# NVIDIA/RAD-MMM

Measured on AMD Instinct MI355X. Metric: mel-frames/sec training step (fwd+bwd), higher is better.
Workload: dtype f32 (f16 hi.hi product + fp8 e4m3 cross terms, fp32 accumulate); 1 GPU; RADTTS flow decoder (configs/RADTTS_model_config.yaml: 8 flows, WN 1024x4, D=1048) fwd+NLL+bwd; batch_per_gpu=32, n_mel=80, frames=800, global_batch=32, parallelism=dp1, includes_optimizer=False

## Files before the change

include/radmmm_hip.h:

```cpp
#ifndef RADMMM_HIP_H
#define RADMMM_HIP_H

#include <stdint.h>

#ifdef __cplusplus
extern "C" {
#endif

#define RADMMM_ABI_VERSION 4

typedef void* radmmm_stream_t;

const char* radmmm_last_error(void);
int radmmm_abi_version(void);

enum { RADMMM_ACT_NONE = 0, RADMMM_ACT_SOFTPLUS = 1, RADMMM_ACT_RELU = 2, RADMMM_ACT_LEAKY = 3 };
enum { RADMMM_SCALE_TANH = 0, RADMMM_SCALE_EXP = 1, RADMMM_SCALE_SIGMOID = 2, RADMMM_SCALE_TRANSLATE = 3 };

#define RADMMM_SPLIT_F16 0
#define RADMMM_SPLIT_X8A 1
#define RADMMM_SPLIT_X8B 2
typedef struct { int fmt; int x8_exp; int32_t* sat_flag;
                 void* lo16;
} radmmm_split_opts;
// ... 82 lines not shown
                        float* gz, int ldz, int rows, int D, int h, radmmm_stream_t stream);

int radmmm_squeeze_rows(const float* in , float* out, int B, int C, int T, int g, int ld, int col0,
                        radmmm_stream_t stream);
int radmmm_unsqueeze_rows(const float* gout, float* gin , int B, int C, int T, int g, int ld, int col0,
                          radmmm_stream_t stream);

int radmmm_affine_coupling_fwd(const float* O, int ldo, const float* z, int ldz,
                               float* zout, float* log_s, int rows, int h, int scaling,
                               radmmm_stream_t stream);
int radmmm_affine_coupling_bwd(const float* O, int ldo, const float* z, int ldz,
                               const float* gzout, const float* glog_s,
                               float* gO, float* gz, int rows, int h, int scaling,
                               radmmm_stream_t stream);

int radmmm_dact_mul(const float* g, int ldg, const float* saved, int lds, float* y, int ldy,
                    int rows, int cols, int dact, int rowscale, int T, const int32_t* lens,
                    int taps, int dil,
                    void* yh, void* yl, int ldyh, float yscale ,
                    const radmmm_split_opts* so , radmmm_stream_t stream);

int radmmm_colsum(const float* X, int ldx, float* out, float* scratch, int rows, int cols,
                  int row_weight, int T, const int32_t* lens, int taps, int dil, int square,
                  radmmm_stream_t stream);
int64_t radmmm_colsum_scratch_floats(int rows, int cols);

int radmmm_masked_reduce(const float* x, int B, int C, int T, int64_t sb, int64_t sc, int64_t st,
                         const int32_t* lens, int mode, float* out, float* scratch,
                         radmmm_stream_t stream);
int64_t radmmm_masked_reduce_scratch_floats(int B, int C, int T);
int radmmm_masked_reduce_bwd(const float* x, int B, int C, int T, int64_t sb, int64_t sc,
                             int64_t st, const int32_t* lens, int mode, const float* coef,
                             float* gx, radmmm_stream_t stream);

int radmmm_fused_add_tanh_sigmoid_multiply(const float* a, const float* b, int ld, float* y,
                                           int ldy, int rows, int n, radmmm_stream_t stream);

int radmmm_pq_spline_fwd(const float* x, int ldx, const float* q, int ldq, float* y, int ldy,
                         float* logj_sum, int rows, int h, int K, radmmm_stream_t stream);
int radmmm_pq_spline_bins(const float* x, int ldx, const float* q, int ldq, int32_t* bins, float* edge_l, float* edge_r,
                          int rows, int h, int K, radmmm_stream_t stream);
int radmmm_pq_spline_inv(const float* y, int ldy, const float* q, int ldq, float* x, int ldx, int rows, int h, int K,
                         radmmm_stream_t stream);
int radmmm_pq_spline_bwd(const float* x, int ldx, const float* q, int ldq, const float* gy,
                         int ldgy, const float* glogj, float* gx, int ldgx, float* gq, int ldgq,
                         int rows, int h, int K, radmmm_stream_t stream);

int radmmm_film_fwd(const float* h2, int ldh, const float* c1, int ldc, const float* x1r, int ldx,
                    const float* mean, const float* invstd, const float* w, const float* b,
                    float* out, int ldo, int rows, int C, int use_bn, radmmm_stream_t stream);
int radmmm_film_bwd(const float* h2, int ldh, const float* c1, int ldc, const float* gout, int ldg,
                    const float* mean, const float* invstd, const float* w, const float* b,
                    float n_valid, int T, const int32_t* lens, float* gh2, int ldgh, float* gc1,
                    int ldgc, float* gx1r, int ldgx, float* gw, float* gb, float* scratch, int rows,
                    int C, int use_bn, radmmm_stream_t stream);
int64_t radmmm_film_bwd_scratch_floats(int rows, int C);
int radmmm_film_bwd_sums(const float* h2, int ldh, const float* c1, int ldc, const float* gout, int ldg,
                         const float* mean, const float* invstd, const float* w, const float* b, float* gw, float* gb,
                         float* scratch, int rows, int C, radmmm_stream_t stream);
int radmmm_film_bwd_apply(const float* h2, int ldh, const float* c1, int ldc, const float* gout, int ldg,
                          const float* mean, const float* invstd, const float* w, const float* b, float n_valid, int T,
                          const int32_t* lens, float* gh2, int ldgh, float* gc1, int ldgc, float* gx1r, int ldgx,
                          const float* scratch, int rows, int C, radmmm_stream_t stream);

int radmmm_attn_fwd(const float* Q, const float* Kx, const float* prior, const int32_t* in_lens,
                    float* attn, float* logprob, int B, int T1, int T2, int Ca, float temp,
// ... 223 lines not shown
```

rad_mmm_amd/_lib.py:

```python
from __future__ import annotations

import ctypes as C
import os
from typing import Optional

import torch

_HERE = os.path.dirname(os.path.abspath(__file__))
LIB_PATH = os.environ.get("RADMMM_LIB_PATH") or os.path.join(_HERE, "libradmmm_hip.so")



def debug_env(name: str, default: Optional[str] = None) -> Optional[str]:
    if os.environ.get("RADMMM_DEBUG", "0") in ("", "0"):
        return default
    return os.environ.get(name, default)


ACT_NONE, ACT_SOFTPLUS, ACT_RELU, ACT_LEAKY = 0, 1, 2, 3
SCALE = {"tanh": 0, "exp": 1, "sigmoid": 2, "translate": 3}
ACT = {"none": 0, "softplus": 1, "relu": 2, "leaky_relu": 3}


class RadmmmError(RuntimeError):
# ... 6 lines not shown
        ("a_item_stride", C.c_int64),
        ("B", C.c_void_p), ("ldb", C.c_int), ("b_tap_stride", C.c_int64), ("b_layout", C.c_int),
        ("C", C.c_void_p), ("ldc", C.c_int),
        ("M", C.c_int), ("N", C.c_int), ("K", C.c_int),
        ("taps", C.c_int), ("dil", C.c_int), ("sign", C.c_int),
        ("T", C.c_int),
        ("lens", C.c_void_p),
        ("a_mask_mode", C.c_int),
        ("bias", C.c_void_p),
        ("pconv", C.c_int), ("premask", C.c_int), ("postmask", C.c_int),
        ("ratio_taps", C.c_int), ("ratio_dil", C.c_int),
        ("add", C.c_void_p), ("ldadd", C.c_int),
        ("dact_src", C.c_void_p), ("lddact", C.c_int), ("dact", C.c_int),
        ("rowscale", C.c_int),
        ("act", C.c_int),
        ("C2", C.c_void_p), ("ldc2", C.c_int), ("c2_accum", C.c_int),
        ("Ch", C.c_void_p), ("Cl", C.c_void_p), ("ldch", C.c_int), ("ch_scale", C.c_float),
        ("C2h", C.c_void_p), ("C2l", C.c_void_p), ("ldc2h", C.c_int), ("c2h_scale", C.c_float),
        ("split_fmt", C.c_int), ("ch_x8_exp", C.c_int), ("c2h_x8_exp", C.c_int),
        ("sat_flag", C.c_void_p),
        ("Clo", C.c_void_p),
        ("colsum_out", C.c_void_p), ("colsum_scratch", C.c_void_p),
        ("dact_h", C.c_void_p), ("dact_x", C.c_void_p), ("lddact_h", C.c_int), ("dact_x8_exp", C.c_int),
        ("c2_src", C.c_void_p * 3), ("n_c2_src", C.c_int),
    ]


class CsItem(C.Structure):
    _fields_ = [("part", C.c_void_p), ("out", C.c_void_p), ("nparts", C.c_int), ("cols", C.c_int)]


class DactItem(C.Structure):
    _fields_ = [("saved", C.c_void_p), ("yh", C.c_void_p), ("yl", C.c_void_p), ("ylo16", C.c_void_p), ("part", C.c_void_p)]


class SplitOpts(C.Structure):
    _fields_ = [("fmt", C.c_int), ("x8_exp", C.c_int), ("sat_flag", C.c_void_p), ("lo16", C.c_void_p)]


SPLIT_F16, SPLIT_X8A, SPLIT_X8B = 0, 1, 2


def split_opts(fmt: int = 0, x8_exp: int = 0, sat_flag: Optional[torch.Tensor] = None, lo16: Optional[torch.Tensor] = None):
    return C.byref(SplitOpts(fmt, x8_exp, sat_flag.data_ptr() if sat_flag is not None else None,
                             lo16.data_ptr() if lo16 is not None else None))


class RowGemmH3Desc(C.Structure):
    _fields_ = [
        ("base", RowGemmDesc),
        ("Ah", C.c_void_p), ("Al", C.c_void_p), ("lda_h", C.c_int),
        ("Bh", C.c_void_p), ("Bl", C.c_void_p), ("ldb_h", C.c_int), ("b_tap_stride_h", C.c_int64),
        ("acc_scale", C.c_float),
        ("nprod", C.c_int),
        ("a8_exp", C.c_int), ("b8_exp", C.c_int),
        ("extra_tap", C.c_int), ("extra_a_rows", C.c_int),
    ]


class WnItem(C.Structure):
    _fields_ = [("v", C.c_void_p), ("g", C.c_void_p), ("Wh", C.c_void_p), ("Wl", C.c_void_p), ("inv_norm", C.c_void_p),
                ("Cout", C.c_int), ("Cin", C.c_int), ("taps", C.c_int), ("ldk", C.c_int), ("perm_split", C.c_int),
                ("off_lo", C.c_int), ("off_hi", C.c_int)]


class TpItem(C.Structure):
# ... 16 lines not shown


def _load() -> C.CDLL:
    if not os.path.exists(LIB_PATH):
        raise ImportError(
            f"{LIB_PATH} not found: build it with `python -c 'import __graft_entry__ as g; g.build()'` "
            "or rad_mmm_amd/csrc/build.sh (hipcc --offload-arch=gfx950). rad_mmm_amd has no fallback path.")
    lib = C.CDLL(LIB_PATH)
    lib.radmmm_last_error.restype = C.c_char_p
    lib.radmmm_abi_version.restype = C.c_int
    lib.radmmm_gemm_cu_slots.restype = C.c_int
    lib.radmmm_gemm_cu_slots.argtypes = []
    if lib.radmmm_abi_version() != 4:
        raise ImportError("libradmmm_hip.so ABI version mismatch")
    i, i64, p = C.c_int, C.c_int64, C.c_void_p
    f = C.c_float
    so = C.POINTER(SplitOpts)
    sig = {
        "radmmm_rowgemm_f32": [C.POINTER(RowGemmDesc), p],
        "radmmm_wgrad_f32": [C.POINTER(WgradDesc), p],
        "radmmm_rowgemm_h3": [C.POINTER(RowGemmH3Desc), p],
        "radmmm_weightnorm_fwd": [p, p, p, p, i, i, i, i, i, i, i, p],
        "radmmm_weightnorm_bwd": [p, p, p, p, i, i64, p, p, i, i, i, i, i, i, i, p, p],
        "radmmm_wn_input_fwd": [p, i, p, i, p, i, i, i, i, p, p, so, p],
        "radmmm_wn_input_bwd": [p, i, p, i, i, p, i, i, i, i, p],
        "radmmm_squeeze_rows": [p, p, i, i, i, i, i, i, p],
        "radmmm_unsqueeze_rows": [p, p, i, i, i, i, i, i, p],
        "radmmm_affine_coupling_fwd": [p, i, p, i, p, p, i, i, i, p],
        "radmmm_affine_coupling_bwd": [p, i, p, i, p, p, p, p, i, i, i, p],
        "radmmm_dact_mul": [p, i, p, i, p, i, i, i, i, i, i, p, i, i, p, p, i, f, so, p],
        "radmmm_colsum": [p, i, p, p, i, i, i, i, p, i, i, i, p],
        "radmmm_masked_reduce": [p, i, i, i, i64, i64, i64, p, i, p, p, p],
        "radmmm_masked_reduce_bwd": [p, i, i, i, i64, i64, i64, p, i, p, p, p],
        "radmmm_fused_add_tanh_sigmoid_multiply": [p, p, i, p, i, i, i, p],
        "radmmm_film_fwd": [p, i, p, i, p, i, p, p, p, p, p, i, i, i, i, p],
        "radmmm_film_bwd": [p, i, p, i, p, i, p, p, p, p, f, i, p, p, i, p, i, p, i, p, p, p, i, i, i, p],
        "radmmm_film_bwd_sums": [p, i, p, i, p, i, p, p, p, p, p, p, p, i, i, p],
        "radmmm_film_bwd_apply": [p, i, p, i, p, i, p, p, p, p, f, i, p, p, i, p, i, p, i, p, i, i, p],
        "radmmm_split_f16": [p, i, p, p, i, i, i, f, so, p],
        "radmmm_transpose_split_act": [p, i, i, i, i, i, i, p, i, f, p, p, p, p, i, p],
        "radmmm_wgrad_h3_tiles": [i, i, i],
        "radmmm_wgrad_rm_tiles": [i, i, i],
        "radmmm_wgrad_rm": [p, p, i, p, p, i, i, i, p, i, p, i, i64, i, i, i, i, i, f, p],
        "radmmm_wgrad_rm8": [p, p, i, i, p, p, i, i, i, i, p, i, p, i, i64, i, i, i, i, i, f, p],
        "radmmm_wgrad_rmh": [p, i, p, i, i, i, p, i, p, i, i64, i, i, i, i, i, f, p],
        "radmmm_betabinom_prior": [i, i, C.c_double, p, p],
        "radmmm_prior_zoom_batch": [p, i, p, i, i, p],
        "radmmm_energy_average": [p, p, i, i, i, i, p],
        "radmmm_lu_weight_fwd": [p, p, p, p, p, i, p, i, i, p, p],
        "radmmm_lu_weight_bwd": [p, p, p, p, p, i, p, i, i, p, p, p, p, p],
        "radmmm_instnorm_fwd": [p, i, p, p, p, i, p, p, p, i, i, i, f, i, p],
        "radmmm_instnorm_bwd": [p, i, p, i, p, i, p, p, p, p, i, p, p, p, i, i, i, i, p],
        "radmmm_pq_spline_inv": [p, i, p, i, p, i, i, i, i, p],
        "radmmm_sumsq": [p, i64, p, p],
        "radmmm_radam_step": [p, p, p, p, i64, p, f, f, f, f, f, i, p],
        "radmmm_transpose_split_act_colsum": [p, i, i, i, i, i, i, p, i, f, p, p, p, p, i, p, i, i, i, p],
        "radmmm_colsum_final": [p, p, i, i, p],
        "radmmm_colsum_final_multi": [C.POINTER(CsItem), i, p], "radmmm_rowgemm_h3_colsum_rows": [C.POINTER(RowGemmH3Desc)],
        "radmmm_dact_mul_transposed": [p, i, p, i, i, i, i, i, i, i, f, p, p, i, so, p, p, i, p, p],
        "radmmm_dact_mul_rows": [p, i, p, i, i, i, i, i, i, p, i, i, f, p, p, i, so, p, p],
        "radmmm_dact_mul_rows_multi": [p, i, C.POINTER(DactItem), i, i, i, i, i, i, f, i, so, p],
        "radmmm_lstm_fwd": [p, p, p, p, p, p, p, p, i, i, i, p],
        "radmmm_stream_create_masked": [i, C.POINTER(C.c_void_p)],
        "radmmm_stream_destroy": [p],
        "radmmm_ctc_monotonic": [p, p, p, p, p, p, i, i, i, p],
        "radmmm_lstm_bwd": [p, p, p, p, p, p, p, p, i, i, i, p, p],
# ... 25 lines not shown
        "radmmm_wg_start_split": [p, i, i, i, p, p, p, i, p, p, i, i, p, i, i, p],
        "radmmm_wg_gate_split": [p, i, p, i, i, p, p, i, i, p, i, i, p],
        "radmmm_wg_res_skip_split": [p, i, p, i, p, i, p, p, i, i, i, i, p, i, i, p],
        "radmmm_wg_end_coupling": [p, i, p, p, p, p, i, i, i, i, p, i, i, p],
        "radmmm_wg_ungroup": [p, i, i, i, p, i64, p, i, i, p],
        "radmmm_wg_group_audio": [p, i64, p, i, i, p, i, i, p],
        "radmmm_wg_mix_fwd": [p, i, i, i, p, p, i, i, p],
        "radmmm_wg_end_coupling_fwd": [p, i, p, p, p, i, i, i, i, p, i, p, p, i, i, p],
        "radmmm_wg_nll_parts": [p, i, i, p, p, i, i, p, p],
        "radmmm_wg_coupling_bwd": [p, i, p, p, p, i, p, i, i, i, i, p, i, p, p, i, p, i, i, p],
        "radmmm_wg_gate_bwd": [p, i, p, i, i, p, i, p, i, i, p, i, i, p],
        "radmmm_wg_coupling_bwd_split": [p, i, p, p, p, i, p, i, i, i, i, p, i, p, p, i, p, p, i, i, f, p, p, i, i, p],
        "radmmm_wg_gate_bwd_split": [p, i, p, i, i, p, i, p, i, p, p, i, i, i, f, p, p, i, i, p],
        "radmmm_wg_start_bwd": [p, i, p, p, i, i, i, i, p, i, i, p],
        "radmmm_wg_outer_reduce": [p, i, i, p, i, i, p, p, p, i, i, p],
        "radmmm_wg_inv_logdet": [p, p, i, p, p, p],
        "radmmm_wg_ungroup_cond": [p, i, p, i64, p, i, i, i, i, p],
        "radmmm_synth_durations": [p, i64, p, i, i, i, p, p, p, p],
        "radmmm_synth_regulate": [p, i64, i, i, i, p, p, i, i, p, i, p],
        "radmmm_synth_f0_stats": [p, i64, p, i64, p, i, i, p, i, p],
        "radmmm_synth_f0_apply": [p, i64, p, i64, p, i64, p, i, i, p, i, p, p, p, p, p, p],
        "radmmm_collate_unpack_pad": [p, i, p, p, p, p, i, i, i, f, p],
        "radmmm_collate_mel": [p, p, p, p, p, p, i, i, i, i, i, f, i, p],
        "radmmm_collate_tracks": [p, p, p, p, p, p, p, p, p, p, p, p, p, p, p, i, i, i, i, f, i, i, p],
    }
    missing = [n for n in sig if not hasattr(lib, n)]
    if missing:
        raise ImportError(f"libradmmm_hip.so lacks symbols {missing}: rebuild it")
    for name, args in sig.items():
        fn = getattr(lib, name)
        fn.argtypes = args
        fn.restype = C.c_int
    for name, args in {"radmmm_colsum_scratch_floats": [i, i], "radmmm_rowgemm_h3_colsum_scratch_floats": [i, i],
                       "radmmm_masked_reduce_scratch_floats": [i, i, i],
                       "radmmm_mas_scratch_bytes": [i, i, i], "radmmm_ctc_monotonic_scratch_floats": [i, i, i],
                       "radmmm_film_bwd_scratch_floats": [i, i],
                       "radmmm_stft_mel_scratch_floats": [i, i, i, i, i],
                       "radmmm_collate_scratch_floats": [i, i, i, i, i],
                       "radmmm_lstm_scratch_bytes": [i, i, i], "radmmm_lstm_hseq_bytes": [i, i, i],
                       "radmmm_wg_outer_reduce_scratch_floats": [i, i, i],
                       "radmmm_sumsq_scratch_floats": []}.items():
        fn = getattr(lib, name)
        fn.argtypes = args
        fn.restype = C.c_int64
    return lib


lib = _load()


def check(rc: int, what: str) -> None:
    if rc != 0:
        raise RadmmmError(f"{what} failed ({rc}): {lib.radmmm_last_error().decode()}")


def stream() -> int:
    return torch.cuda.current_stream().cuda_stream


def ptr(t: Optional[torch.Tensor]) -> Optional[int]:
    if t is None:
        return None
    if not t.is_cuda:
        raise RadmmmError("rad_mmm_amd ops need GPU tensors (there is no CPU path)")
    if t.dtype is torch.bfloat16:
        raise RadmmmError("a bfloat16 tensor reached the fp32 C ABI (an autocast region upstream?): cast it to float")
    return t.data_ptr()
# ... 105 lines not shown
```

rad_mmm_amd/csrc/elementwise.hip:

```cpp
#include <math.h>
#include <stdlib.h>

#include "common.h"
#include "split_pack.h"

namespace {

using radmmm::block_sum;
using radmmm::wave_sum;

__device__ __forceinline__ int perm_col(int ci, int perm_split, int off_lo, int off_hi) {
  return ci < perm_split ? ci + off_lo : ci - perm_split + off_hi;
}

__global__ __launch_bounds__(256) void weightnorm_fwd_kernel(
    const float* __restrict__ v, const float* __restrict__ g, float* __restrict__ W,
    float* __restrict__ inv_norm, int Cout, int Cin, int taps, int ldw, int perm_split,
    int off_lo, int off_hi) {
  __shared__ float sh[17];
  const int co = blockIdx.x;
  const int n = Cin * taps;
  const float* vr = v + (long long)co * n;
  float ss = 0.f;
  for (int i = threadIdx.x; i < n; i += blockDim.x) ss = fmaf(vr[i], vr[i], ss);
// ... 459 lines not shown
  for (int i = threadIdx.x; i < n; i += blockDim.x) acc += part[i];
  acc = block_sum(acc, sh);
  if (threadIdx.x == 0) out[0] = acc;
}
__global__ __launch_bounds__(256) void masked_reduce_bwd_kernel(
    const float* __restrict__ x, int B, int C, int T, long long sb, long long sc, long long st,
    const int* __restrict__ lens, int mode, const float* __restrict__ coef,
    float* __restrict__ gx) {
  const long long total = (long long)B * C * T;
  const bool c_inner = sc < st;
  const float cf = coef[0];
  for (long long i = blockIdx.x * (long long)blockDim.x + threadIdx.x; i < total;
       i += (long long)gridDim.x * blockDim.x) {
    int b, c, t;
    if (c_inner) {
      c = (int)(i % C);
      const long long j = i / C;
      t = (int)(j % T);
      b = (int)(j / T);
    } else {
      t = (int)(i % T);
      const long long j = i / T;
      c = (int)(j % C);
      b = (int)(j / C);
    }
    const int len = lens ? lens[b] : T;
    const long long off = b * sb + c * sc + t * st;
    float v = 0.f;
    if (t < len) v = mode ? 2.f * cf * x[off] : cf;
    gx[off] = v;
  }
}

__global__ __launch_bounds__(256) void fatsm_kernel(const float* __restrict__ a,
                                                    const float* __restrict__ b, int ld,
                                                    float* __restrict__ y, int ldy, int rows, int n) {
  const long long total = (long long)rows * n;
  for (long long i = blockIdx.x * (long long)blockDim.x + threadIdx.x; i < total;
       i += (long long)gridDim.x * blockDim.x) {
    const int r = (int)(i / n), c = (int)(i - (long long)r * n);
    const float t = a[(long long)r * ld + c] + b[(long long)r * ld + c];
    const float s = a[(long long)r * ld + n + c] + b[(long long)r * ld + n + c];
    y[(long long)r * ldy + c] = tanhf(t) * (1.f / (1.f + expf(-s)));
  }
}

inline int grid_for(long long total, int block = 256, int cap = 256 * 8) {
  long long g = (total + block - 1) / block;
  if (g > cap) g = cap;
  if (g < 1) g = 1;
  return (int)g;
}

}

#define ST(s) static_cast<hipStream_t>(s)

extern "C" int radmmm_weightnorm_fwd(const float* v, const float* g, float* W, float* inv_norm,
                                     int Cout, int Cin, int taps, int ldw, int perm_split,
                                     int off_lo, int off_hi, radmmm_stream_t stream) {
  RADMMM_REQUIRE(v && g && W && inv_norm, "weightnorm_fwd: null pointer");
  RADMMM_REQUIRE(Cout > 0 && Cin > 0 && taps > 0 && ldw >= Cin, "weightnorm_fwd: bad dims");
  hipLaunchKernelGGL(weightnorm_fwd_kernel, dim3(Cout), dim3(256), 0, ST(stream), v, g, W, inv_norm,
                     Cout, Cin, taps, ldw, perm_split, off_lo, off_hi);
  return radmmm::check_launch("weightnorm_fwd");
}
// ... 191 lines not shown
}

extern "C" int radmmm_colsum_final(const float* part, float* out, int nparts, int cols, radmmm_stream_t stream) {
  RADMMM_REQUIRE(part && out && nparts > 0 && cols > 0, "colsum_final: bad arguments");
  hipLaunchKernelGGL(colsum_final_kernel, dim3((cols + 63) / 64), dim3(1024), 0, ST(stream), part, out, nparts, cols);
  return radmmm::check_launch("colsum_final");
}

extern "C" int64_t radmmm_masked_reduce_scratch_floats(int, int, int) { return MR_BLOCKS; }

extern "C" int radmmm_masked_reduce(const float* x, int B, int C, int T, int64_t sb, int64_t sc,
                                    int64_t st, const int32_t* lens, int mode, float* out,
                                    float* scratch, radmmm_stream_t stream) {
  RADMMM_REQUIRE(x && out && scratch, "masked_reduce: null pointer");
  RADMMM_REQUIRE(B > 0 && C > 0 && T > 0, "masked_reduce: bad dims");
  const int nb = grid_for((long long)B * C * T, 256, MR_BLOCKS);
  hipLaunchKernelGGL(masked_reduce_kernel, dim3(nb), dim3(256), 0, ST(stream), x, B, C, T,
                     (long long)sb, (long long)sc, (long long)st, lens, mode, scratch);
  hipLaunchKernelGGL(reduce_final_kernel, dim3(1), dim3(256), 0, ST(stream), scratch, nb, out);
  return radmmm::check_launch("masked_reduce");
}

extern "C" int radmmm_masked_reduce_bwd(const float* x, int B, int C, int T, int64_t sb, int64_t sc,
                                        int64_t st, const int32_t* lens, int mode, const float* coef,
                                        float* gx, radmmm_stream_t stream) {
  RADMMM_REQUIRE(coef && gx && (x || mode == 0), "masked_reduce_bwd: null pointer");
  RADMMM_REQUIRE(B > 0 && C > 0 && T > 0, "masked_reduce_bwd: bad dims");
  hipLaunchKernelGGL(masked_reduce_bwd_kernel, dim3(grid_for((long long)B * C * T)), dim3(256), 0,
                     ST(stream), x, B, C, T, (long long)sb, (long long)sc, (long long)st, lens, mode,
                     coef, gx);
  return radmmm::check_launch("masked_reduce_bwd");
}

extern "C" int radmmm_fused_add_tanh_sigmoid_multiply(const float* a, const float* b, int ld, float* y,
                                                      int ldy, int rows, int n,
                                                      radmmm_stream_t stream) {
  RADMMM_REQUIRE(a && b && y, "fused_add_tanh_sigmoid_multiply: null pointer");
  RADMMM_REQUIRE(rows > 0 && n > 0 && ld >= 2 * n && ldy >= n, "fused_add_tanh_sigmoid_multiply: bad dims");
  hipLaunchKernelGGL(fatsm_kernel, dim3(grid_for((long long)rows * n)), dim3(256), 0, ST(stream), a, b,
                     ld, y, ldy, rows, n);
  return radmmm::check_launch("fused_add_tanh_sigmoid_multiply");
}

namespace {
template <bool INVERSE>
__global__ __launch_bounds__(256) void squeeze_rows_kernel(float* __restrict__ in, float* __restrict__ out, int C, int T,
                                                           int g, int Tg, int ld, int col0) {
  __shared__ float tile[32][65];
  const int b = blockIdx.z, c0 = blockIdx.y * 32, t0 = blockIdx.x * 64;
  const int tid = threadIdx.x;
  const int rows_per_tile = 64 / g, cols_per_row = 32 * g;
  const long long row0 = (long long)b * Tg + t0 / g;
  if (!INVERSE) {
#pragma unroll
    for (int i = 0; i < 8; ++i) {
      const int c = c0 + i * 4 + (tid >> 6), t = t0 + (tid & 63);
      tile[i * 4 + (tid >> 6)][tid & 63] = (c < C && t < Tg * g) ? in[((long long)b * C + c) * T + t] : 0.f;
    }
    __syncthreads();
#pragma unroll
    for (int j = 0; j < 8; ++j) {
      const int e = tid + 256 * j;
      const int r = e / cols_per_row, cc = e - r * cols_per_row;
      const int c = cc / g, k = cc - c * g;
      if (c0 + c < C && t0 / g + r < Tg) out[(row0 + r) * ld + col0 + (c0 + c) * g + k] = tile[c][r * g + k];
    }
// ... 41 lines not shown
```

rad_mmm_amd/loss.py:

```python
from __future__ import annotations

from typing import Optional

import torch
from torch import nn
import torch.nn.functional as F

from . import ops
from .common import SequenceLength
from ._trace import traced


def compute_flow_loss(z, log_det_W_list, log_s_list, n_elements, n_dims, lens32, sigma=1.0):
    log_s_total = None
    for log_s in log_s_list:
        s = ops.masked_sum(log_s, lens32)
        log_s_total = s if log_s_total is None else log_s_total + s
    log_det_W_total = 0.0
    if len(log_det_W_list):
        log_det_W_total = torch.stack(list(log_det_W_list)).sum() * n_elements
    prior_NLL = ops.masked_sumsq(z, lens32) / (2 * sigma * sigma)
    loss = prior_NLL - log_s_total - log_det_W_total
    denom = n_elements * n_dims
    return loss / denom, prior_NLL / denom


class AttentionCTCLoss(nn.Module):

    def __init__(self, blank_logprob=-1):
        super().__init__()
        self.blank_logprob = blank_logprob

    def forward(self, attn_logprob, in_lens, out_lens, in_lens_host=None, out_lens_host=None):
        padded = F.pad(attn_logprob, (1, 0), value=self.blank_logprob)[:, 0]
        B, _, C = padded.shape
        cls = torch.arange(C, device=padded.device)
        lp = padded.masked_fill(cls[None, None, :] > in_lens[:, None, None], -1e4)
        lp = torch.log_softmax(lp, -1)
        if lp.is_cuda and C - 1 <= 511:
            loss = ops.CTCMonotonicFn.apply(lp, in_lens.to(torch.int32).contiguous(), out_lens.to(torch.int32).contiguous())
        else:
            targets = cls[1:][None].expand(B, -1)
            loss = F.ctc_loss(lp.transpose(0, 1), targets, out_lens if out_lens_host is None else out_lens_host,
                              in_lens if in_lens_host is None else in_lens_host, blank=0, reduction="none", zero_infinity=True)
        return (loss / in_lens.clamp_min(1).to(loss.dtype)).sum() / B

# ... 16 lines not shown
                 ctc_loss_weight=0.1):
        super().__init__()
        self.attn_ctc_loss = AttentionCTCLoss(blank_logprob=CTC_blank_logprob)
        self.attn_bin_loss = AttentionBinarizationLoss()
        self.kl_loss_start_iter = kl_loss_start_iter
        self.binarization_loss_weight = binarization_loss_weight
        self.ctc_loss_weight = ctc_loss_weight

    def forward(self, attn, attn_soft, attn_logprob, global_step, in_lens, out_lens, in_lens_host=None, out_lens_host=None):
        loss_dict = {"loss_ctc": (self.attn_ctc_loss(attn_logprob, in_lens, out_lens, in_lens_host, out_lens_host),
                                  self.ctc_loss_weight)}
        if global_step > self.kl_loss_start_iter:
            loss_dict["binarization_loss"] = (self.attn_bin_loss(attn, attn_soft), self.binarization_loss_weight)
        else:
            loss_dict["binarization_loss"] = (0.0, self.binarization_loss_weight)
        return loss_dict


class RADTTSLoss(nn.Module):

    def __init__(self, sigma=1.0, n_group_size=1, CTC_blank_logprob=-1, kl_loss_start_iter=5000,
                 binarization_loss_weight=1.0, ctc_loss_weight=0.1):
        super().__init__()
        self.sigma = sigma
        self.n_group_size = n_group_size
        self.attn_loss = AttentionLoss(CTC_blank_logprob, kl_loss_start_iter, binarization_loss_weight,
                                       ctc_loss_weight)

    @traced("loss")
    def forward(self, model_output, in_lens: Optional[SequenceLength], out_lens: SequenceLength, global_step):
        loss_dict = {}
        if len(model_output["z_mel"]):
            g = self.n_group_size
            n_elements = torch.div(out_lens.lengths.sum(), g, rounding_mode="floor")
            lens32 = torch.div(out_lens.lengths, g, rounding_mode="floor").to(torch.int32)
            n_dims = model_output["z_mel"].size(1)
            loss_mel, loss_prior_mel = compute_flow_loss(
                model_output["z_mel"], model_output["log_det_W_list"], model_output["log_s_list"], n_elements,
                n_dims, lens32, self.sigma)
            loss_dict["loss_mel"] = (loss_mel, 1.0)
            loss_dict["loss_prior_mel"] = (loss_prior_mel, 0.0)
        if "attn_logprob" in model_output:
            loss_dict.update(self.attn_loss(model_output["attn"], model_output["attn_soft"],
                                            model_output["attn_logprob"], global_step, in_lens.lengths,
                                            out_lens.lengths, getattr(in_lens, "lengths_host", None),
                                            getattr(out_lens, "lengths_host", None)))
        return loss_dict


class RADMMMLoss(RADTTSLoss):

    def __init__(self, sigma=1.0, n_group_size=1, CTC_blank_logprob=-1, kl_loss_start_iter=5000,
                 binarization_loss_weight=1.0, ctc_loss_weight=0.1, use_spk_embed_reg=False,
                 use_accent_embed_reg=False, reg_loss_config=None, use_spk_accent_cross_covariance=False,
                 cross_reg_loss_config=None):
        super().__init__(sigma, n_group_size, CTC_blank_logprob, kl_loss_start_iter, binarization_loss_weight,
                         ctc_loss_weight)
        self.use_spk_embed_reg = bool(use_spk_embed_reg)
        self.use_accent_embed_reg = bool(use_accent_embed_reg)
        self.use_spk_accent_cross_covariance = bool(use_spk_accent_cross_covariance)
        self.reg_loss_config = reg_loss_config
        self.cross_reg_loss_config = cross_reg_loss_config


class AttributeBCELoss(nn.Module):

    def __init__(self, prefix: Optional[str] = None, weight=1.0):
        super().__init__()
        self.prefix, self.weight = prefix, weight

    def forward(self, model_output, in_lens, out_lens, global_step, mask=None):
        target, prediction = model_output["x"], model_output["x_hat"]
# ... 56 lines not shown
```

rad_mmm_amd/ops.py:

```python
from __future__ import annotations

import collections
import math
import os
import types
from typing import List, Optional, Sequence, Tuple

import torch

from . import _lib as L
from ._lib import (ACT, SCALE, lib, check, ptr, stream, rowgemm, wgrad, f32c, amp_fwd, amp_bwd, split_opts, SPLIT_F16,
                   SPLIT_X8A, SPLIT_X8B)

ZLD = 160


def _empty(*shape, like: torch.Tensor) -> torch.Tensor:
    return torch.empty(*shape, device=like.device, dtype=torch.float32)


def round_up(x: int, m: int) -> int:
    return (x + m - 1) // m * m


# ... 348 lines not shown
    @amp_fwd
    def forward(ctx, x, lens, mode):
        assert x.dim() == 3 and x.dtype == torch.float32
        B, C, T = x.shape
        out = _empty(1, like=x)
        scratch = _empty(int(lib.radmmm_masked_reduce_scratch_floats(B, C, T)), like=x)
        sb, sc, st = x.stride()
        check(lib.radmmm_masked_reduce(ptr(x), B, C, T, sb, sc, st, ptr(lens), mode, ptr(out), ptr(scratch),
                                       stream()), "masked_reduce")
        ctx.save_for_backward(x, lens)
        ctx.mode = mode
        return out.view(())

    @staticmethod
    @amp_bwd
    def backward(ctx, g):
        x, lens = ctx.saved_tensors
        B, C, T = x.shape
        gx = torch.empty_like(x)
        assert gx.stride() == x.stride()
        coef = g.reshape(1).contiguous().float()
        sb, sc, st = x.stride()
        check(lib.radmmm_masked_reduce_bwd(ptr(x), B, C, T, sb, sc, st, ptr(lens), ctx.mode, ptr(coef), ptr(gx),
                                           stream()), "masked_reduce_bwd")
        return gx, None, None


def masked_sum(x, lens):
    return MaskedReduceFn.apply(x, lens, 0)


def masked_sumsq(x, lens):
    return MaskedReduceFn.apply(x, lens, 1)


def fused_add_tanh_sigmoid_multiply(a: torch.Tensor, b: torch.Tensor, n_channels: int) -> torch.Tensor:
    rows, ld = a.shape
    y = _empty(rows, n_channels, like=a)
    check(lib.radmmm_fused_add_tanh_sigmoid_multiply(ptr(a), ptr(b), ld, ptr(y), n_channels, rows, n_channels,
                                                     stream()), "fused_add_tanh_sigmoid_multiply")
    return y


class ConvNormFn(torch.autograd.Function):

    @staticmethod
    @amp_fwd
    def forward(ctx, meta, x, v, g, bias, lens):
        B, T, dil = meta["B"], meta["T"], meta["dil"]
        partial, mask_out, act = meta["partial"], meta["mask_out"], meta["act"]
        Cout, Cin, taps = v.shape
        N = B * T
        assert x.shape[0] == N and x.shape[1] >= Cin and x.shape[1] % 4 == 0 and x.is_contiguous()
        if g is not None:
            W, inv = weightnorm_fwd(v, g)
        else:
            ldw = round_up(Cin, 4)
            W = torch.zeros(taps, Cout, ldw, device=x.device, dtype=torch.float32)
            W[:, :, :Cin] = v.permute(2, 0, 1)
            inv = None
        ldy = round_up(Cout, 4)
        y = torch.zeros(N, ldy, device=x.device, dtype=torch.float32) if ldy != Cout else _empty(N, ldy, like=x)
        rowgemm(A=x, lda=x.shape[1], B=W, ldb=W.shape[2], b_tap_stride=W.stride(0), b_layout=0, C=y, ldc=ldy,
                M=N, N=Cout, K=Cin, taps=taps, dil=dil, sign=1, T=T, lens=lens, a_mask_mode=1 if partial else 0,
                bias=bias, pconv=1 if partial else 0, ratio_taps=taps, ratio_dil=dil,
                postmask=1 if mask_out else 0, act=act)
# ... 1132 lines not shown
```

Measured before the change: 709,300 mel-frames/s.

## Fuse flow NLL loss reductions and backward into table-driven kernels

```diff
diff --git a/include/radmmm_hip.h b/include/radmmm_hip.h
--- a/include/radmmm_hip.h
+++ b/include/radmmm_hip.h
@@ -138,6 +138,30 @@
 int radmmm_masked_reduce_bwd(const float* x, int B, int C, int T, int64_t sb, int64_t sc,
                              int64_t st, const int32_t* lens, int mode, const float* coef,
                              float* gx, radmmm_stream_t stream);
+
+#define RADMMM_NLL_MAX 16
+typedef struct radmmm_nll_item {
+  const float* x;
+  float* gx;
+  int64_t sb, sc, st;
+  int C;
+  int pad_;
+} radmmm_nll_item;
+typedef struct radmmm_flow_nll_table {
+  radmmm_nll_item t[RADMMM_NLL_MAX + 1];
+  const float* log_det_W[RADMMM_NLL_MAX];
+  float* g_log_det_W[RADMMM_NLL_MAX];
+  const void* lens;
+  const int64_t* n_elements;
+  int n_log_s, n_log_det_W;
+  int lens_i64;
+  int B, T, g, n_dims;
+  float inv_two_sigma_sq;
+} radmmm_flow_nll_table;
+int radmmm_flow_nll_fwd(const radmmm_flow_nll_table* tab, float* out, radmmm_stream_t stream);
+int64_t radmmm_flow_nll_out_floats(void);
+int radmmm_flow_nll_bwd(const radmmm_flow_nll_table* tab, const float* out, const float* g_loss,
+                        const float* g_prior, radmmm_stream_t stream);
 
 int radmmm_fused_add_tanh_sigmoid_multiply(const float* a, const float* b, int ld, float* y,
                                            int ldy, int rows, int n, radmmm_stream_t stream);
diff --git a/rad_mmm_amd/_lib.py b/rad_mmm_amd/_lib.py
--- a/rad_mmm_amd/_lib.py
+++ b/rad_mmm_amd/_lib.py
@@ -62,6 +62,21 @@
 
 class DactItem(C.Structure):
     _fields_ = [("saved", C.c_void_p), ("yh", C.c_void_p), ("yl", C.c_void_p), ("ylo16", C.c_void_p), ("part", C.c_void_p)]
+
+
+NLL_MAX = 16
+
+
+class NllItem(C.Structure):
+    _fields_ = [("x", C.c_void_p), ("gx", C.c_void_p), ("sb", C.c_int64), ("sc", C.c_int64), ("st", C.c_int64),
+                ("C", C.c_int), ("pad_", C.c_int)]
+
+
+class FlowNllTable(C.Structure):
+    _fields_ = [("t", NllItem * (NLL_MAX + 1)), ("log_det_W", C.c_void_p * NLL_MAX), ("g_log_det_W", C.c_void_p * NLL_MAX),
+                ("lens", C.c_void_p), ("n_elements", C.c_void_p), ("n_log_s", C.c_int), ("n_log_det_W", C.c_int),
+                ("lens_i64", C.c_int), ("B", C.c_int), ("T", C.c_int), ("g", C.c_int), ("n_dims", C.c_int),
+                ("inv_two_sigma_sq", C.c_float)]
 
 
 class SplitOpts(C.Structure):
@@ -144,6 +159,8 @@
         "radmmm_colsum": [p, i, p, p, i, i, i, i, p, i, i, i, p],
         "radmmm_masked_reduce": [p, i, i, i, i64, i64, i64, p, i, p, p, p],
         "radmmm_masked_reduce_bwd": [p, i, i, i, i64, i64, i64, p, i, p, p, p],
+        "radmmm_flow_nll_fwd": [C.POINTER(FlowNllTable), p, p],
+        "radmmm_flow_nll_bwd": [C.POINTER(FlowNllTable), p, p, p, p],
         "radmmm_fused_add_tanh_sigmoid_multiply": [p, p, i, p, i, i, i, p],
         "radmmm_film_fwd": [p, i, p, i, p, i, p, p, p, p, p, i, i, i, i, p],
         "radmmm_film_bwd": [p, i, p, i, p, i, p, p, p, p, f, i, p, p, i, p, i, p, i, p, p, p, i, i, i, p],
@@ -235,7 +252,7 @@
         fn.argtypes = args
         fn.restype = C.c_int
     for name, args in {"radmmm_colsum_scratch_floats": [i, i], "radmmm_rowgemm_h3_colsum_scratch_floats": [i, i],
-                       "radmmm_masked_reduce_scratch_floats": [i, i, i],
+                       "radmmm_masked_reduce_scratch_floats": [i, i, i], "radmmm_flow_nll_out_floats": [],
                        "radmmm_mas_scratch_bytes": [i, i, i], "radmmm_ctc_monotonic_scratch_floats": [i, i, i],
                        "radmmm_film_bwd_scratch_floats": [i, i],
                        "radmmm_stft_mel_scratch_floats": [i, i, i, i, i],
diff --git a/rad_mmm_amd/csrc/elementwise.hip b/rad_mmm_amd/csrc/elementwise.hip
--- a/rad_mmm_amd/csrc/elementwise.hip
+++ b/rad_mmm_amd/csrc/elementwise.hip
@@ -515,6 +515,157 @@
   }
 }
 
+constexpr int NLL_BLOCKS = 256;
+constexpr int NLL_HEAD = 4;
+
+__device__ __forceinline__ long long nll_raw_len(const radmmm_flow_nll_table& m, int b) {
+  return m.lens_i64 ? static_cast<const long long*>(m.lens)[b] : (long long)static_cast<const int*>(m.lens)[b];
+}
+__device__ __forceinline__ bool nll_live(const radmmm_flow_nll_table& m, int b, int t) {
+  return (long long)(t + 1) * m.g <= nll_raw_len(m, b);
+}
+struct NllWalk {
+  int in, mid, b;
+  int n0, n1;
+  int s_in, s_mid, s_b;
+  long long off, off_step, k1, k2;
+  long long left;
+  bool c_inner;
+  __device__ __forceinline__ void init(const radmmm_nll_item& it, int B, int T, long long first, unsigned step) {
+    c_inner = it.sc < it.st;
+    n0 = c_inner ? it.C : T;
+    n1 = c_inner ? T : it.C;
+    const long long s0 = c_inner ? it.sc : it.st, s1 = c_inner ? it.st : it.sc;
+    const long long total = (long long)B * it.C * T;
+    if (total < (1ll << 31)) {
+      const unsigned f = (unsigned)first, j = f / (unsigned)n0;
+      in = (int)(f - j * (unsigned)n0);
+      b = (int)(j / (unsigned)n1);
+      mid = (int)(j - (unsigned)b * (unsigned)n1);
+      left = f < (unsigned)total ? ((unsigned)total - f - 1) / step + 1 : 0;
+    } else {
+      const long long j = first / n0;
+      in = (int)(first - j * n0);
+      b = (int)(j / n1);
+      mid = (int)(j - (long long)b * n1);
+      left = first < total ? (total - first - 1) / step + 1 : 0;
+    }
+    const unsigned sj = step / (unsigned)n0;
+    s_in = (int)(step - sj * (unsigned)n0);
+    s_b = (int)(sj / (unsigned)n1);
+    s_mid = (int)(sj - (unsigned)s_b * (unsigned)n1);
+    off = b * it.sb + in * s0 + mid * s1;
+    off_step = s_b * it.sb + s_in * s0 + s_mid * s1;
+    k1 = s1 - n0 * s0;
+    k2 = it.sb - n1 * s1;
+  }
+  __device__ __forceinline__ int t() const { return c_inner ? mid : in; }
+  __device__ __forceinline__ void next() {
+    in += s_in;
+    off += off_step;
+    if (in >= n0) { in -= n0; ++mid; off += k1; }
+    mid += s_mid;
+    if (mid >= n1) { mid -= n1; ++b; off += k2; }
+    b += s_b;
+  }
+};
+__global__ __launch_bounds__(256) void flow_nll_partial_kernel(const radmmm_flow_nll_table m, float* __restrict__ part) {
+  __shared__ float sh[17];
+  const radmmm_nll_item& it = m.t[blockIdx.y];
+  const bool square = blockIdx.y == 0;
+  const float* __restrict__ x = it.x;
+  NllWalk w;
+  w.init(it, m.B, m.T, (long long)blockIdx.x * blockDim.x + threadIdx.x, gridDim.x * blockDim.x);
+  float acc = 0.f;
+  for (; w.left >= 4; w.left -= 4) {
+    float v[4];
+#pragma unroll
+    for (int k = 0; k < 4; ++k) {
+      const float xv = x[w.off];
+      v[k] = nll_live(m, w.b, w.t()) ? xv : 0.f;
+      w.next();
+    }
+#pragma unroll
+    for (int k = 0; k < 4; ++k) acc += square ? v[k] * v[k] : v[k];
+  }
+  for (; w.left > 0; --w.left) {
+    const float xv = x[w.off];
+    const float v = nll_live(m, w.b, w.t()) ? xv : 0.f;
+    acc += square ? v * v : v;
+    w.next();
+  }
+  acc = block_sum(acc, sh);
+  if (threadIdx.x == 0) part[blockIdx.y * NLL_BLOCKS + blockIdx.x] = acc;
+}
+__global__ __launch_bounds__(256) void flow_nll_final_kernel(const radmmm_flow_nll_table m, float* __restrict__ out) {
+  static_assert(NLL_BLOCKS == 256, "four partials per lane");
+  __shared__ float ssum[RADMMM_NLL_MAX + 1], sw[RADMMM_NLL_MAX];
+  __shared__ long long slen[4];
+  const float* part = out + NLL_HEAD;
+  const int lane = threadIdx.x & 63, wv = threadIdx.x >> 6;
+  for (int k = wv; k <= m.n_log_s; k += 4) {
+    const float* p = part + k * NLL_BLOCKS + lane;
+    const float p0 = p[0], p1 = p[64], p2 = p[128], p3 = p[192];
+    const float s = radmmm::wave_sum((p0 + p1) + (p2 + p3));
+    if (lane == 0) ssum[k] = s;
+  }
+  if ((int)threadIdx.x < m.n_log_det_W) sw[threadIdx.x] = m.log_det_W[threadIdx.x][0];
+  long long ls = 0;
+  if (!m.n_elements)
+    for (int b = threadIdx.x; b < m.B; b += blockDim.x) ls += nll_raw_len(m, b);
+#pragma unroll
+  for (int o = 32; o > 0; o >>= 1) ls += __shfl_xor(ls, o, 64);
+  if (lane == 0) slen[wv] = ls;
+  __syncthreads();
+  if (threadIdx.x == 0) {
+    const long long n_el = m.n_elements ? m.n_elements[0] : ((slen[0] + slen[1]) + (slen[2] + slen[3])) / m.g;
+    float s_total = 0.f;
+    for (int k = 1; k <= m.n_log_s; ++k) s_total = k == 1 ? ssum[1] : s_total + ssum[k];
+    const float prior = __fmul_rn(ssum[0], m.inv_two_sigma_sq);
+    float loss = prior - s_total;
+    if (m.n_log_det_W) {
+      float w = 0.f;
+      for (int j = 0; j < m.n_log_det_W; ++j) w += sw[j];
+      loss = loss - __fmul_rn(w, (float)n_el);
+    }
+    const float denom = (float)(n_el * m.n_dims);
+    out[0] = __fdiv_rn(loss, denom);
+    out[1] = __fdiv_rn(prior, denom);
+    out[2] = denom;
+    out[3] = (float)n_el;
+  }
+}
+__global__ __launch_bounds__(256) void flow_nll_bwd_kernel(const radmmm_flow_nll_table m, const float* __restrict__ out,
+                                                           const float* __restrict__ g_loss,
+                                                           const float* __restrict__ g_prior) {
+  const float denom = out[2];
+  const float a = g_loss ? __fdiv_rn(g_loss[0], denom) : 0.f;
+  const float gp = g_prior ? (g_loss ? a + __fdiv_rn(g_prior[0], denom) : __fdiv_rn(g_prior[0], denom)) : a;
+  const int k = blockIdx.y;
+  const radmmm_nll_item& it = m.t[k];
+  if (it.gx) {
+    const float cf = k == 0 ? 2.f * __fmul_rn(gp, m.inv_two_sigma_sq) : -a;
+    const float* __restrict__ x = it.x;
+    float* __restrict__ gx = it.gx;
+    NllWalk w;
+    w.init(it, m.B, m.T, (long long)blockIdx.x * blockDim.x + threadIdx.x, gridDim.x * blockDim.x);
+    if (k == 0) {
+      for (; w.left > 0; --w.left) {
+        const float xv = x[w.off];
+        gx[w.off] = nll_live(m, w.b, w.t()) ? __fmul_rn(cf, xv) : 0.f;
+        w.next();
+      }
+    } else {
+      for (; w.left > 0; --w.left) {
+        gx[w.off] = nll_live(m, w.b, w.t()) ? cf : 0.f;
+        w.next();
+      }
+    }
+  }
+  if (blockIdx.x == 0 && k == 0 && (int)threadIdx.x < m.n_log_det_W && m.g_log_det_W[threadIdx.x])
+    m.g_log_det_W[threadIdx.x][0] = __fmul_rn(-a, out[3]);
+}
+
 __global__ __launch_bounds__(256) void fatsm_kernel(const float* __restrict__ a,
                                                     const float* __restrict__ b, int ld,
                                                     float* __restrict__ y, int ldy, int rows, int n) {
@@ -772,6 +923,44 @@
   return radmmm::check_launch("masked_reduce_bwd");
 }
 
+extern "C" int64_t radmmm_flow_nll_out_floats(void) { return NLL_HEAD + (int64_t)(RADMMM_NLL_MAX + 1) * NLL_BLOCKS; }
+
+static int flow_nll_check(const radmmm_flow_nll_table* m, const char* what, bool bwd, long long* max_total) {
+  RADMMM_REQUIRE(m, "%s: null table", what);
+  RADMMM_REQUIRE(m->n_log_s >= 0 && m->n_log_s <= RADMMM_NLL_MAX && m->n_log_det_W >= 0 && m->n_log_det_W <= RADMMM_NLL_MAX,
+                 "%s: at most %d log_s tensors and %d log_det_W scalars per call", what, RADMMM_NLL_MAX, RADMMM_NLL_MAX);
+  RADMMM_REQUIRE(m->lens && m->B > 0 && m->T > 0 && m->g > 0 && m->n_dims > 0, "%s: bad dims", what);
+  *max_total = 0;
+  for (int k = 0; k <= m->n_log_s; ++k) {
+    const bool read = bwd ? (k == 0 && m->t[0].gx) : true;
+    RADMMM_REQUIRE((m->t[k].x || !read) && m->t[k].C > 0, "%s: bad tensor %d", what, k);
+    const long long total = (long long)m->B * m->t[k].C * m->T;
+    *max_total = total > *max_total ? total : *max_total;
+  }
+  for (int j = 0; j < m->n_log_det_W && !bwd; ++j) RADMMM_REQUIRE(m->log_det_W[j], "%s: null log_det_W %d", what, j);
+  return 0;
+}
+
+extern "C" int radmmm_flow_nll_fwd(const radmmm_flow_nll_table* tab, float* out, radmmm_stream_t stream) {
+  long long max_total;
+  if (int rc = flow_nll_check(tab, "flow_nll_fwd", false, &max_total)) return rc;
+  RADMMM_REQUIRE(out, "flow_nll_fwd: null pointer");
+  hipLaunchKernelGGL(flow_nll_partial_kernel, dim3(NLL_BLOCKS, tab->n_log_s + 1), dim3(256), 0, ST(stream), *tab,
+                     out + NLL_HEAD);
+  hipLaunchKernelGGL(flow_nll_final_kernel, dim3(1), dim3(256), 0, ST(stream), *tab, out);
+  return radmmm::check_launch("flow_nll_fwd");
+}
+
+extern "C" int radmmm_flow_nll_bwd(const radmmm_flow_nll_table* tab, const float* out, const float* g_loss,
+                                   const float* g_prior, radmmm_stream_t stream) {
+  long long max_total;
+  if (int rc = flow_nll_check(tab, "flow_nll_bwd", true, &max_total)) return rc;
+  RADMMM_REQUIRE(out && (g_loss || g_prior), "flow_nll_bwd: null pointer");
+  hipLaunchKernelGGL(flow_nll_bwd_kernel, dim3(grid_for(max_total, 256, NLL_BLOCKS), tab->n_log_s + 1), dim3(256), 0, ST(stream),
+                     *tab, out, g_loss, g_prior);
+  return radmmm::check_launch("flow_nll_bwd");
+}
+
 extern "C" int radmmm_fused_add_tanh_sigmoid_multiply(const float* a, const float* b, int ld, float* y,
                                                       int ldy, int rows, int n,
                                                       radmmm_stream_t stream) {
diff --git a/rad_mmm_amd/loss.py b/rad_mmm_amd/loss.py
--- a/rad_mmm_amd/loss.py
+++ b/rad_mmm_amd/loss.py
@@ -12,6 +12,12 @@
 
 
 def compute_flow_loss(z, log_det_W_list, log_s_list, n_elements, n_dims, lens32, sigma=1.0):
+    if isinstance(n_dims, int) and ops.flow_nll_fusable(z, log_det_W_list, log_s_list, lens32):
+        n_el = n_elements
+        if isinstance(n_el, int) and not isinstance(n_el, bool):
+            n_el = torch.full((1,), n_el, dtype=torch.int64, device=z.device)
+        if torch.is_tensor(n_el) and n_el.is_cuda and n_el.numel() == 1 and n_el.dtype in (torch.int32, torch.int64):
+            return ops.flow_nll(z, log_det_W_list, log_s_list, lens32, 1, sigma, n_dims, n_el.to(torch.int64))
     log_s_total = None
     for log_s in log_s_list:
         s = ops.masked_sum(log_s, lens32)
@@ -94,12 +100,13 @@
         loss_dict = {}
         if len(model_output["z_mel"]):
             g = self.n_group_size
-            n_elements = torch.div(out_lens.lengths.sum(), g, rounding_mode="floor")
-            lens32 = torch.div(out_lens.lengths, g, rounding_mode="floor").to(torch.int32)
-            n_dims = model_output["z_mel"].size(1)
-            loss_mel, loss_prior_mel = compute_flow_loss(
-                model_output["z_mel"], model_output["log_det_W_list"], model_output["log_s_list"], n_elements,
-                n_dims, lens32, self.sigma)
+            z, ldw, ls = model_output["z_mel"], model_output["log_det_W_list"], model_output["log_s_list"]
+            if ops.flow_nll_fusable(z, ldw, ls, out_lens.lengths):
+                loss_mel, loss_prior_mel = ops.flow_nll(z, ldw, ls, out_lens.lengths, g, self.sigma)
+            else:
+                n_elements = torch.div(out_lens.lengths.sum(), g, rounding_mode="floor")
+                lens32 = torch.div(out_lens.lengths, g, rounding_mode="floor").to(torch.int32)
+                loss_mel, loss_prior_mel = compute_flow_loss(z, ldw, ls, n_elements, z.size(1), lens32, self.sigma)
             loss_dict["loss_mel"] = (loss_mel, 1.0)
             loss_dict["loss_prior_mel"] = (loss_prior_mel, 0.0)
         if "attn_logprob" in model_output:
diff --git a/rad_mmm_amd/ops.py b/rad_mmm_amd/ops.py
--- a/rad_mmm_amd/ops.py
+++ b/rad_mmm_amd/ops.py
@@ -404,6 +404,87 @@
 
 def masked_sumsq(x, lens):
     return MaskedReduceFn.apply(x, lens, 1)
+
+
+def _dense3(x: torch.Tensor) -> bool:
+    expect = 1
+    for s, n in sorted(zip(x.stride(), x.shape)):
+        if n != 1 and s != expect:
+            return False
+        expect *= n
+    return True
+
+
+def flow_nll_fusable(z, log_det_W_list, log_s_list, lens) -> bool:
+    if L.debug_env("RADMMM_FUSED_NLL", "1") == "0":
+        return False
+    if not (torch.is_tensor(z) and z.is_cuda and z.dim() == 3 and z.numel() and torch.is_tensor(lens) and lens.is_cuda
+            and lens.dtype in (torch.int32, torch.int64) and lens.dim() == 1 and lens.shape[0] == z.shape[0]):
+        return False
+    if not 1 <= len(log_s_list) <= L.NLL_MAX or len(log_det_W_list) > L.NLL_MAX:
+        return False
+    for x in (z, *log_s_list):
+        if not (torch.is_tensor(x) and x.is_cuda and x.dtype == torch.float32 and x.dim() == 3 and x.shape[0] == z.shape[0]
+                and x.shape[2] == z.shape[2] and x.shape[1] > 0 and _dense3(x)):
+            return False
+    return all(torch.is_tensor(w) and w.is_cuda and w.dtype == torch.float32 and w.numel() == 1 for w in log_det_W_list)
+
+
+class FlowNLLFn(torch.autograd.Function):
+
+    @staticmethod
+    @amp_fwd
+    def forward(ctx, lens, g, sigma, n_dims, n_elements, n_log_s, z, *rest):
+        log_s, ldw = rest[:n_log_s], rest[n_log_s:]
+        B, _, T = z.shape
+        tab = L.FlowNllTable()
+        for k, x in enumerate((z, *log_s)):
+            it = tab.t[k]
+            it.x, it.C = ptr(x), x.shape[1]
+            it.sb, it.sc, it.st = x.stride()
+        for j, w in enumerate(ldw):
+            tab.log_det_W[j] = ptr(w)
+        tab.lens, tab.lens_i64 = ptr(lens), int(lens.dtype == torch.int64)
+        tab.n_elements = ptr(n_elements)
+        tab.n_log_s, tab.n_log_det_W = len(log_s), len(ldw)
+        tab.B, tab.T, tab.g, tab.n_dims = B, T, int(g), int(n_dims)
+        tab.inv_two_sigma_sq = 1.0 / L.C.c_float(2 * sigma * sigma).value
+        out = _empty(int(lib.radmmm_flow_nll_out_floats()), like=z)
+        check(lib.radmmm_flow_nll_fwd(L.C.byref(tab), ptr(out), stream()), "flow_nll_fwd")
+        ctx.save_for_backward(z, lens, out, n_elements)
+        ctx.table = tab
+        ctx.layouts = [(tuple(x.shape), x.stride()) for x in log_s]
+        ctx.n_ldw = len(ldw)
+        ctx.set_materialize_grads(False)
+        return out[0], out[1]
+
+    @staticmethod
+    @amp_bwd
+    def backward(ctx, g_loss, g_prior):
+        z, lens, out, n_elements = ctx.saved_tensors
+        tab, need = ctx.table, ctx.needs_input_grad[6:]
+        n_log_s = len(ctx.layouts)
+        gz = torch.empty_strided(z.shape, z.stride(), device=z.device, dtype=torch.float32) if need[0] else None
+        gs = [torch.empty_strided(shape, stride, device=z.device, dtype=torch.float32) if need[1 + k] else None
+              for k, (shape, stride) in enumerate(ctx.layouts)]
+        gw = _empty(ctx.n_ldw, like=z) if ctx.n_ldw and any(need[1 + n_log_s:]) else None
+        tab.t[0].x, tab.lens, tab.n_elements = ptr(z), ptr(lens), ptr(n_elements)
+        for k, t in enumerate((gz, *gs)):
+            tab.t[k].gx = ptr(t)
+        for k in range(1, n_log_s + 1):
+            tab.t[k].x = None
+        for j in range(ctx.n_ldw):
+            tab.log_det_W[j] = None
+            tab.g_log_det_W[j] = gw[j].data_ptr() if gw is not None and need[1 + n_log_s + j] else None
+        g_loss, g_prior = (None if t is None else t.float().reshape(1) for t in (g_loss, g_prior))
+        check(lib.radmmm_flow_nll_bwd(L.C.byref(tab), ptr(out), ptr(g_loss), ptr(g_prior), stream()), "flow_nll_bwd")
+        gws = [gw[j] if gw is not None and need[1 + n_log_s + j] else None for j in range(ctx.n_ldw)]
+        return (None,) * 6 + (gz, *gs, *gws)
+
+
+def flow_nll(z, log_det_W_list, log_s_list, lens, g=1, sigma=1.0, n_dims=None, n_elements=None):
+    return FlowNLLFn.apply(lens.contiguous(), g, sigma, z.shape[1] if n_dims is None else n_dims, n_elements,
+                           len(log_s_list), z, *log_s_list, *log_det_W_list)
 
 
 def fused_add_tanh_sigmoid_multiply(a: torch.Tensor, b: torch.Tensor, n_channels: int) -> torch.Tensor:
```

Measured after the change: 715,900 mel-frames/s, median of 6. Within noise of the previous version (+0.9%).
